# zhou-lab/biscuit

Measured on AMD Instinct MI355X. Metric: paired-end reads aligned/sec, higher is better.
Workload: dtype int32

## Files before the change

biscuit_amd/csrc/hip/k_swl.hip:

```cpp
#include <hip/hip_runtime.h>
#include "dev_common.hpp"
#include "wave.hpp"
#include "kernels.h"

#define SWL_ROW_ROR(n) (0x120 + (n))
__device__ __forceinline__ int swl_shl1(int v) { return __builtin_amdgcn_update_dpp(0, v, DPP_ROW_SHR(1), 0xf, 0xf, false); }
__device__ __forceinline__ int swl_row_max(int v)
{
	int t;
	t = __builtin_amdgcn_update_dpp(v, v, SWL_ROW_ROR(1), 0xf, 0xf, false); v = v > t ? v : t;
	t = __builtin_amdgcn_update_dpp(v, v, SWL_ROW_ROR(2), 0xf, 0xf, false); v = v > t ? v : t;
	t = __builtin_amdgcn_update_dpp(v, v, SWL_ROW_ROR(4), 0xf, 0xf, false); v = v > t ? v : t;
	t = __builtin_amdgcn_update_dpp(v, v, SWL_ROW_ROR(8), 0xf, 0xf, false); v = v > t ? v : t;
	return v;
}
__device__ __forceinline__ int swl_row_min(int v)
{
	int t;
	t = __builtin_amdgcn_update_dpp(v, v, SWL_ROW_ROR(1), 0xf, 0xf, false); v = v < t ? v : t;
	t = __builtin_amdgcn_update_dpp(v, v, SWL_ROW_ROR(2), 0xf, 0xf, false); v = v < t ? v : t;
	t = __builtin_amdgcn_update_dpp(v, v, SWL_ROW_ROR(4), 0xf, 0xf, false); v = v < t ? v : t;
	t = __builtin_amdgcn_update_dpp(v, v, SWL_ROW_ROR(8), 0xf, 0xf, false); v = v < t ? v : t;
	return v;
}
__device__ __forceinline__ unsigned int swl_row_or(unsigned int v)
{
	v |= (unsigned int)__builtin_amdgcn_update_dpp((int)v, (int)v, SWL_ROW_ROR(1), 0xf, 0xf, false);
	v |= (unsigned int)__builtin_amdgcn_update_dpp((int)v, (int)v, SWL_ROW_ROR(2), 0xf, 0xf, false);
	v |= (unsigned int)__builtin_amdgcn_update_dpp((int)v, (int)v, SWL_ROW_ROR(4), 0xf, 0xf, false);
	v |= (unsigned int)__builtin_amdgcn_update_dpp((int)v, (int)v, SWL_ROW_ROR(8), 0xf, 0xf, false);
	return v;
}
__device__ __forceinline__ int swl_clamp(int v, int hi) { return v < 0 ? 0 : v > hi ? hi : v; }

template <int SL, bool UNI>
__device__ __forceinline__ int swl_row(int (&H)[SL], int (&E)[SL], const uint32_t (&prof)[SL], int tsh, int cap, int slen,
                                       int oe_del, int e_del, int oe_ins, int e_ins, int col0_e)
{
	int f = 0, mxv = 0, hlast = 0, gl = NEG_BIG, ce = col0_e;
#pragma unroll
	for (int j = 0; j < SL; ++j) hlast = j == slen - 1 ? H[j] : hlast;
	int h = swl_shl1(hlast);
#pragma unroll
	for (int j = 0; j < SL; ++j) {
		if (j < slen) {
			const int s = (int)(int8_t)(prof[j] >> tsh);
			h = swl_clamp(h + s, cap);
			int e = E[j];
			h = h > e ? h : e;
			h = h > f ? h : f;
			mxv = mxv > h ? mxv : h;
			const int hold = H[j];
			H[j] = h;
			e -= e_del;
			int t = h - oe_del;
			e = e > t ? e : t;
			E[j] = e > 0 ? e : 0;
			f -= e_ins;
			t = h - oe_ins;
			f = f > t ? f : t;
			f = f > 0 ? f : 0;
			t += ce; gl = gl > t ? gl : t;
			ce += e_ins;
			h = hold;
		}
	}
	int t;
	t = __builtin_amdgcn_update_dpp(NEG_BIG, gl, DPP_ROW_SHR(1), 0xf, 0xf, false); gl = gl > t ? gl : t;
	t = __builtin_amdgcn_update_dpp(NEG_BIG, gl, DPP_ROW_SHR(2), 0xf, 0xf, false); gl = gl > t ? gl : t;
	t = __builtin_amdgcn_update_dpp(NEG_BIG, gl, DPP_ROW_SHR(4), 0xf, 0xf, false); gl = gl > t ? gl : t;
	t = __builtin_amdgcn_update_dpp(NEG_BIG, gl, DPP_ROW_SHR(8), 0xf, 0xf, false); gl = gl > t ? gl : t;
	int v = __builtin_amdgcn_update_dpp(NEG_BIG, gl, DPP_ROW_SHR(1), 0xf, 0xf, false) - (col0_e - e_ins);
	if (__ballot(v > 0) != 0) {
#pragma unroll
		for (int j = 0; j < SL; ++j) {
			if (j < slen) { H[j] = H[j] > v ? H[j] : v; v -= e_ins; }
		}
	}
	return mxv;
}

template <int SL>
__global__ void __launch_bounds__(256)
k_swl(DevIndex ix, DevScoring sc, const uint8_t *reads, const bsx_sw_job_t *jobs, const int *order, long long n,
      bsx_sw_res_t *res, unsigned long long *bscratch, int bcap)
{
	const int lane = wave_lane(), g = lane >> 4, k = lane & 15;
	const long long wave_id = (long long)blockIdx.x * (blockDim.x >> 6) + (threadIdx.x >> 6), n_waves = (long long)gridDim.x * (blockDim.x >> 6);
	unsigned long long *b = bscratch + ((size_t)wave_id * 4 + g) * (size_t)bcap;
	const int oe_del = sc.o_del + sc.e_del, oe_ins = sc.o_ins + sc.e_ins, e_del = sc.e_del, e_ins = sc.e_ins;
	for (long long q4 = wave_id; q4 * 4 < n; q4 += n_waves) {
		const long long jj = q4 * 4 + g;
		const bool valid = jj < n;
		const int job = valid ? order[jj] : 0;
		bsx_sw_job_t J = jobs[valid ? job : order[0]];
		const int8_t *mat = J.use_ct ? sc.ctmat : sc.gamat;
		int shift = 127, mx = 0;
		for (int a = 0; a < 25; ++a) { const int m = mat[a]; shift = m < shift ? m : shift; mx = m > mx ? m : mx; }
		shift = (int)(uint8_t)(256 - (int)(uint8_t)shift);
		const int cap = 255 - shift;
		bsx_sw_res_t o;
		o.score = 0; o.te = -1; o.qe = -1; o.score2 = -1; o.te2 = -1; o.tb = -1; o.qb = -1;
		int r_score = 0, r_te = -1, r_qe = -1;
		bool run = valid;
		for (int pass = 0; pass < 2; ++pass) {
			const int qlen = pass ? r_qe + 1 : J.qlen, tlen = J.tlen, te_rev = pass ? r_te : -1;
			const int xtra = pass ? (BSX_KSW_XSTOP | r_score) : J.xtra;
			const int minsc = (xtra & BSX_KSW_XSUBO) ? (xtra & 0xffff) : 0x10000;
			const int endsc = (xtra & BSX_KSW_XSTOP) ? (xtra & 0xffff) : 0x10000;
			const int slen = (qlen + 15) >> 4;
			const int slen_s = __builtin_amdgcn_readfirstlane(wave_max_i32(run ? slen : 0));
			const bool uni = __ballot(run && slen != slen_s) == 0;
			int H[SL], E[SL], Hm[SL];
			uint32_t prof[SL];
#pragma unroll
			for (int j = 0; j < SL; ++j) {
				H[j] = E[j] = Hm[j] = 0;
				const int c = j + k * slen;
				int q = 5;
				if (run && j < slen && c < qlen) {
					q = pass ? reads[(long long)J.qoff + (long long)(r_qe - c) * J.qdir] : reads[(long long)J.qoff + (long long)c * J.qdir];
					if (J.qcomp) q = q < 4 ? 3 - q : 4;
				}
				prof[j] = q > 4 ? 0u : ((uint32_t)(uint8_t)mat[q] | (uint32_t)(uint8_t)mat[5 + q] << 8 | (uint32_t)(uint8_t)mat[10 + q] << 16 | (uint32_t)(uint8_t)mat[15 + q] << 24);
			}
			int gmax = 0, te = -1, n_b = 0;
			unsigned long long b_last = 0;
			unsigned int tw = 0;
			bool live = run && tlen > 0;
			int rows = live ? tlen : 0;
			rows = wave_max_i32(rows);
			for (int i = 0; i < rows; ++i) {
				if (!__builtin_amdgcn_readfirstlane(__ballot(live) != 0)) break;
				if (live && i >= tlen) live = false;
				if (live) {
					if ((i & 15) == 0) {
						const int ii = i + k;
						const long long src = (ii <= te_rev) ? (long long)(te_rev - ii) : (long long)ii;
						const unsigned int tb = ii < tlen ? (unsigned int)dev_ref_base(ix.pac, ix.l_pac, J.tpos + src * J.tdir) : 0u;
						tw = swl_row_or(tb << (k << 1));
					}
					const int tsh = (int)((tw >> ((i & 15) << 1)) & 3u) << 3;
					int mxv;
					if (uni) mxv = swl_row<SL, true>(H, E, prof, tsh, cap, slen_s, oe_del, e_del, oe_ins, e_ins, k * slen_s * e_ins);
					else mxv = swl_row<SL, false>(H, E, prof, tsh, cap, slen, oe_del, e_del, oe_ins, e_ins, k * slen * e_ins);
					const int imax = swl_row_max(mxv);
					if (imax >= minsc) {
						if (n_b == 0 || (int)(uint32_t)b_last + 1 != i) { b_last = (unsigned long long)imax << 32 | (uint32_t)i; ++n_b; }
						else if ((int)(b_last >> 32) < imax) b_last = (unsigned long long)imax << 32 | (uint32_t)i;
						if (k == 0) b[n_b - 1] = b_last;
					}
					if (imax > gmax) {
						gmax = imax; te = i;
#pragma unroll
						for (int j = 0; j < SL; ++j) Hm[j] = H[j];
						if (gmax + shift >= 255 || gmax >= endsc) live = false;
					}
				}
			}
			const int score = gmax + shift < 255 ? gmax : 255;
			int qe = -1, score2 = -1, te2 = -1;
			if (run && score != 255) {
				int lm = -1, lj = 0x7fffffff;
#pragma unroll
				for (int j = 0; j < SL; ++j) if (j < slen) { const int c = j + k * slen; if (Hm[j] > lm || (Hm[j] == lm && c < lj)) { lm = Hm[j]; lj = c; } }
				const int m = swl_row_max(lm);
				qe = swl_row_min(lm == m ? lj : 0x7fffffff);
				if (n_b > 0) {
					WAVE_SYNC();
					const int rad = (score + mx - 1) / mx, low = te - rad, high = te + rad;
					int bs = -1, bi = 0x7fffffff;
					for (int x = k; x < n_b; x += 16) {
						const unsigned long long v = b[x];
						const int e = (int)(uint32_t)v, s2 = (int)(v >> 32);
						if ((e < low || e > high) && s2 > bs) { bs = s2; bi = x; }
					}
					const int ms = swl_row_max(bs);
					if (ms >= 0) {
						const int mi = swl_row_min(bs == ms ? bi : 0x7fffffff);
						score2 = ms; te2 = (int)(uint32_t)b[mi];
					}
					WAVE_SYNC();
				}
			}
			if (pass == 0) {
				o.score = score; o.te = te; o.qe = qe; o.score2 = score2; o.te2 = te2;
				r_score = score; r_te = te; r_qe = qe;
				run = run && (J.xtra & BSX_KSW_XSTART) && !((J.xtra & BSX_KSW_XSUBO) && score < (J.xtra & 0xffff)) && qe >= 0;
				if (__ballot(run) == 0) break;
			} else if (run && r_score == score) { o.tb = r_te - te; o.qb = r_qe - qe; }
		}
		if (valid && k == 0) res[job] = o;
	}
}

void launch_swl(hipStream_t st, const DevIndex &ix, const DevScoring &sc, const uint8_t *reads, const bsx_sw_job_t *jobs, const int *order,
                long long n, bsx_sw_res_t *res, unsigned long long *bscratch, int bcap, int blocks, int slen_max)
{
	if (slen_max <= 10) hipLaunchKernelGGL((k_swl<10>), dim3(blocks), dim3(256), 0, st, ix, sc, reads, jobs, order, n, res, bscratch, bcap);
	else hipLaunchKernelGGL((k_swl<16>), dim3(blocks), dim3(256), 0, st, ix, sc, reads, jobs, order, n, res, bscratch, bcap);
}
```

biscuit_amd/csrc/hip/kernels.h:

```cpp
#pragma once
#include <hip/hip_runtime.h>
#include "dev_common.hpp"
#include "seed_core.hpp"
#include "seed_tab.hpp"
#include "ctr_layout.hpp"

void launch_seed(hipStream_t st, int grid, const DevIndex &ix, const uint8_t *reads, const bsx_seed_task_t *tasks, int n_tasks, const SeedParams &P,
                 DevIntv *scratch, int list_cap, int mem_cap, DevIntv *out, unsigned long long out_cap, unsigned long long *out_cursor,
                 long long *task_off, int *task_n, unsigned int *task_cursor, unsigned long long *counters,
                 int quota, unsigned int *slab_busy, int n_slabs, int trip_budget, int prof = 0, uint32_t *qpack = nullptr, unsigned long long direct_off = ~0ull);
void launch_seedt(hipStream_t st, int grid, const DevIndex &ix, const uint8_t *reads, const bsx_seed_task_t *tasks, int n_tasks, const SeedParams &P,
                  DevIntv *scratch, int list_cap, int mem_cap, DevIntv *out, unsigned long long out_cap, unsigned long long *out_cursor,
                  long long *task_off, int *task_n, unsigned int *task_cursor, unsigned long long *counters,
                  int quota, unsigned int *slab_busy, int n_slabs, int trip_budget, int prof = 0, uint32_t *qpack = nullptr, unsigned long long direct_off = ~0ull);
size_t seedt_pack_bytes(long long n_tasks);
void launch_gather_lists(hipStream_t st, const DevIntv *src, const long long *off, const int *cnt, const long long *which, const long long *dst_off, long long n_list, DevIntv *dst);
int seedtab_build(hipStream_t st, const DevIndex &ix, int parent, int K, void *table);
void launch_bwt_planes(hipStream_t st, uint32_t *bwt, unsigned long long n_words);
void launch_sa(hipStream_t st, int grid, const DevIndex &ix, const bsx_sa_job_t *jobs, long long n, uint64_t *pos, unsigned long long *counters);
void launch_extend(hipStream_t st, const DevIndex &ix, const DevScoring &sc, const uint8_t *reads, const bsx_ext_job_t *jobs, const int *order,
                   long long n, bsx_ext_res_t *res, int qcap, int nc, int n_cu);
size_t extend_hbm_row_bytes(int qcap);
void launch_extend_hbm(hipStream_t st, const DevIndex &ix, const DevScoring &sc, const uint8_t *reads, const bsx_ext_job_t *jobs, const int *order,
                       long long n, bsx_ext_res_t *res, int qcap, int blocks, void *rows);
size_t global_hbm_row_bytes(int qcap);
void launch_global_hbm(hipStream_t st, const DevIndex &ix, const DevScoring &sc, const uint8_t *reads, const bsx_glb_job_t *jobs, const int *order,
                       long long n, bsx_glb_res_t *res, uint32_t *pool, uint8_t *zscratch, size_t zstride, int qcap, int blocks,
                       bsx_glb_tag_t *tags, char *md_pool, unsigned long long md_cap, unsigned long long *md_cursor, void *rows, bsx_glb_ctx_t *ctx = nullptr);
void launch_sw(hipStream_t st, const DevIndex &ix, const DevScoring &sc, const uint8_t *reads, const bsx_sw_job_t *jobs, const int *order,
               long long n, bsx_sw_res_t *res, unsigned long long *bscratch, int bcap, int blocks, int nc);
void launch_swl(hipStream_t st, const DevIndex &ix, const DevScoring &sc, const uint8_t *reads, const bsx_sw_job_t *jobs, const int *order,
                long long n, bsx_sw_res_t *res, unsigned long long *bscratch, int bcap, int blocks, int slen_max);
void launch_global(hipStream_t st, const DevIndex &ix, const DevScoring &sc, const uint8_t *reads, const bsx_glb_job_t *jobs, const int *order,
                   long long n, bsx_glb_res_t *res, uint32_t *pool, uint8_t *zscratch, size_t zstride, int qcap, int nc, int blocks, int wpb,
                   bsx_glb_tag_t *tags = nullptr, char *md_pool = nullptr, unsigned long long md_cap = 0, unsigned long long *md_cursor = nullptr, int tcap = 0,
                   bsx_glb_ctx_t *ctx = nullptr);
void launch_qc(hipStream_t st, const DevIndex &ix, const uint8_t *reads, long long reads_len, const bsx_qc_job_t *jobs, long long n, const uint32_t *pool,
               unsigned long long *table, int n_cu);
#define COV_LDS_BINS_MAX 512
size_t cov_n_tiles(long long l_pac);
size_t cov_diff_entries(long long l_pac);
size_t cov_mask_words(long long l_pac);
void launch_cov_add(hipStream_t st, int n_cu, void *diff, long long l_pac, const bsx_qc_job_t *jobs, long long n, const uint32_t *pool, long long pool_len);
void launch_cov_paint(hipStream_t st, int n_cu, uint32_t *mask, long long l_pac, const long long *beg_end, long long n);
void launch_cov_sums(hipStream_t st, int n_cu, const void *diff, long long n_tiles, void *tsum);
void launch_cov_max(hipStream_t st, int n_cu, const DevIndex &ix, const void *diff, const void *carry, long long n_tiles, int *gmax);
void launch_cov_count(hipStream_t st, int n_cu, const DevIndex &ix, const void *diff, const void *carry, long long n_tiles, const uint32_t *m_top,
                      const uint32_t *m_bot, int lds_bins, int flush_tiles, unsigned long long *bins, long long nb);
#define METH_FLUSH_TILES_MAX 1024
size_t meth_n_tiles(long long l_pac);
size_t meth_state_entries(long long l_pac);
void launch_meth_add(hipStream_t st, const DevIndex &ix, const uint8_t *reads, long long reads_len, const bsx_meth_job_t *jobs, long long n,
                     const uint32_t *pool, long long pool_len, void *state, int n_cu);
void launch_meth_tables(hipStream_t st, int n_cu, const DevIndex &ix, const void *state, long long n_tiles, int flush_tiles, unsigned long long *out);
struct MdSlot { unsigned long long claim, ord, k0, k1; };
enum { MD_CTR_TAKEN = 0, MD_CTR_OPEN = 1, MD_CTR_LOST = 2 };
enum { MD_RES_FIRST = 0, MD_RES_DUP = 1, MD_RES_OPEN = 2, MD_RES_SKIP = 3, MD_RES_FULL = 4 };
void launch_md_init(hipStream_t st, MdSlot *T, unsigned long long n_slots);
void launch_md_round(hipStream_t st, MdSlot *T, unsigned long long n_slots, const bsx_markdup_key_t *keys, long long n, unsigned long long first,
                     unsigned salt, int bits, uint8_t *res, unsigned long long *slot, unsigned long long *ctr);
void launch_md_rehash(hipStream_t st, const MdSlot *old, unsigned long long n_old, MdSlot *T, unsigned long long n_slots, unsigned long long *ctr);
#define SORT_SCAN_BLOCK 2048
size_t sort_n_tiles(long long n);
size_t sort_n_scan_blocks(long long n);
void launch_sort_bits(hipStream_t st, const unsigned long long *keys, long long n, unsigned long long *bits);
// ... 75 lines not shown
```

biscuit_amd/csrc/hip/shim.hip:

```cpp
#include <hip/hip_runtime.h>
#include <stdio.h>
#include <stdlib.h>
#include <string.h>
#include <time.h>
#include <algorithm>
#include <vector>
#include <mutex>
#include <atomic>
#include "devbuf.hpp"
#include "kernels.h"
#include "index_build.h"
#include "tune.h"
#include "ext_pk_bound.h"

#define HIPCHK(x) do { hipError_t e_ = (x); if (e_ != hipSuccess) { fprintf(stderr, "[bsx-hip] %s failed: %s (%s:%d)\n", #x, hipGetErrorString(e_), __FILE__, __LINE__); return BSX_E_NODEVICE; } } while (0)

#define BSX_LANES 6
enum KTime { KT_SEED = 0, KT_K3 = 1, KT_EXTEND = 2, KT_SW = 3, KT_GLOBAL = 4, KT_TIER1 = 5, KT_TIERS_LATER = 6, KT_SEED_OTHER = 7, KT_N = 8 };
struct Lane {
	hipStream_t st = nullptr;
	hipEvent_t ev_seed_done = nullptr, ev_regions_done = nullptr;
	hipStream_t st_hi = nullptr;
	hipEvent_t ev_timed_begin = nullptr, ev_timed_end = nullptr;
	hipEvent_t ev_seed2_begin = nullptr, ev_seed2_end = nullptr;
// ... 1583 lines not shown
		else if (!launch_swl16_batch(L.st_hi, d->n_cu, d->ix, L.sc, (const uint8_t*)L.reads.p, (const bsx_sw_job_t*)L.jobs.p, (bsx_sw_res_t*)L.res.p, (unsigned int)n, L.scratch.p))
			return BSX_E_ARG;
		HIPCHK(hipGetLastError());
		D2H(L.st_hi, res, L.res.p, (size_t)n * sizeof(bsx_sw_res_t));
		return BSX_OK;
	}
	std::vector<int> order[4];
	int max_tlen = 1, slen_max = 1;
	const bool use_swl = true;
	std::vector<int> key;
	for (int64_t i = 0; i < n; ++i) {
		const bsx_sw_job_t &j = jobs[i];
		if (j.qlen <= 0 || j.tlen < 0) { fprintf(stderr, "[bsx-hip] sw job %lld: invalid\n", (long long)i); return BSX_E_ARG; }
		const int p = (j.xtra & BSX_KSW_XBYTE) ? 16 : 8, Q = (j.qlen + p - 1) / p * p;
		if (Q > 3072) { fprintf(stderr, "[bsx-hip] sw job %lld: query %d beyond kernel limit (3072)\n", (long long)i, j.qlen); return BSX_E_ARG; }
		max_tlen = std::max(max_tlen, j.tlen);
		if (use_swl && p == 16 && Q <= 256) { order[3].push_back((int)i); slen_max = std::max(slen_max, Q / 16); }
		else order[Q <= 256 ? 0 : Q <= 1024 ? 1 : 2].push_back((int)i);
	}
	if (order[3].size() > 4) {
		const int NK = 17 * 2048;
		std::vector<int> cnt((size_t)NK + 1, 0), sorted(order[3].size());
		auto keyof = [&](int i) { const bsx_sw_job_t &j = jobs[i]; return ((j.qlen + 15) >> 4) * 2048 + (2047 - std::min(j.tlen, 2047)); };
		for (int i : order[3]) ++cnt[(size_t)keyof(i) + 1];
		for (int x = 0; x < NK; ++x) cnt[(size_t)x + 1] += cnt[(size_t)x];
		for (int i : order[3]) sorted[(size_t)cnt[(size_t)keyof(i)]++] = i;
		order[3].swap(sorted);
	}
	int rc;
	const int blocks_cap = d->n_cu * 8;
	if ((rc = L.jobs.reserve((size_t)n * sizeof(bsx_sw_job_t))) != BSX_OK) return rc;
	if ((rc = L.res.reserve((size_t)n * sizeof(bsx_sw_res_t))) != BSX_OK) return rc;
	if ((rc = L.aux.reserve((size_t)n * 4 + 64)) != BSX_OK) return rc;
	if ((rc = L.scratch.reserve((size_t)blocks_cap * 4 * 4 * (size_t)max_tlen * 8)) != BSX_OK) return rc;
	const bool tr_sw = bsx_phases() != 0;
	const double ts0 = tr_sw ? bsx_now_s() : 0;
	H2D(L.st_hi, L.jobs.p, jobs, (size_t)n * sizeof(bsx_sw_job_t));
	size_t off = 0;
	for (int c = 0; c < 4; ++c) if (!order[c].empty()) {
		H2D(L.st_hi, (int*)L.aux.p + off, order[c].data(), order[c].size() * 4);
		off += order[c].size();
	}
	HIPCHK(hipEventRecord(L.ev_timed_begin, L.st_hi));
	off = 0;
	for (int c = 0; c < 4; ++c) if (!order[c].empty()) {
		const long long m = (long long)order[c].size();
		if (c == 3) {
			const int blocks = (int)std::min<long long>((m + 15) / 16, blocks_cap);
			launch_swl(L.st_hi, d->ix, L.sc, (const uint8_t*)L.reads.p, (const bsx_sw_job_t*)L.jobs.p, (const int*)L.aux.p + off, m,
			           (bsx_sw_res_t*)L.res.p, (unsigned long long*)L.scratch.p, max_tlen, blocks, slen_max);
		} else {
			const int blocks = (int)std::min<long long>((m + 3) / 4, blocks_cap);
			launch_sw(L.st_hi, d->ix, L.sc, (const uint8_t*)L.reads.p, (const bsx_sw_job_t*)L.jobs.p, (const int*)L.aux.p + off, m,
			          (bsx_sw_res_t*)L.res.p, (unsigned long long*)L.scratch.p, max_tlen, blocks, c == 0 ? 4 : c == 1 ? 16 : 48);
		}
		off += order[c].size();
	}
	HIPCHK(hipEventRecord(L.ev_timed_end, L.st_hi));
	const double ts1 = tr_sw ? bsx_now_s() : 0;
	if ((rc = finish_timed(L, KT_SW)) != BSX_OK) return rc;
	const double ts2 = tr_sw ? bsx_now_s() : 0;
	D2H(L.st_hi, res, L.res.p, (size_t)n * sizeof(bsx_sw_res_t));
	if (tr_sw) { float ms = 0; (void)hipEventElapsedTime(&ms, L.ev_timed_begin, L.ev_timed_end);
		fprintf(stderr, "[M::sw_batch] %lld jobs: upload %.3f s, waited %.3f s for the kernels (%.3f s on the device), download %.3f s\n", (long long)n, ts1 - ts0, ts2 - ts1, ms * 1e-3, bsx_now_s() - ts2); }
	return BSX_OK;
}

static int lane_regions_dedup(bsx_device_t *d, int lane, const bsx_opt_t *opt, int64_t n_reads, int per_read, int32_t *out_n, uint8_t *out_idx,
                              int64_t *long_off = nullptr, uint16_t **long_idx = nullptr, int64_t *long_cap = nullptr)
{
	if (!d || !d->has_index) return BSX_E_NODEVICE;
	if (!opt || !out_n || !out_idx || per_read < 1) return BSX_E_ARG;
	Lane &L = d->lane[lane];
	if (n_reads == 0) return BSX_OK;
	if (n_reads * per_read != L.rb_tasks) { fprintf(stderr, "[bsx-hip] regions_dedup: %lld reads x %d strand searches, but the last regions batch had %lld\n", (long long)n_reads, per_read, (long long)L.rb_tasks); return BSX_E_ARG; }
	HIPCHK(hipSetDevice(d->ordinal));
	int rc;
	const int64_t n = L.rb_tasks;
	const size_t cap = (size_t)dedup_cap();
	const bool with_long = long_off && long_idx && long_cap && per_read <= 4 && bsx_tune_long("long_dedup", 1) != 0;
	const size_t pool_cap = with_long ? (size_t)L.rs.used_main + 64 : 0;
	const size_t o_idx = (size_t)n_reads * 4, o_list = (o_idx + (size_t)n_reads * cap + 15) & ~(size_t)15, o_off = o_list + (size_t)n_reads * 8, o_cnt = o_off + (size_t)n_reads * 8, o_pool = o_cnt + 16;
	if ((rc = L.dd.reserve(with_long ? o_pool + pool_cap * 2 + 64 : o_idx + (size_t)n_reads * cap + 64)) != BSX_OK) return rc;
// ... 36 lines not shown
	if (p1 <= p0) { *n_jobs = 0; return BSX_OK; }
	if (!bsx_tune_long("msw_plan", 0)) return BSX_OK;
	if (!L.ddl.valid || L.ddl.n_reads != n_reads || L.ddl.per_read != per_read || n_reads * per_read != L.rb_tasks) return BSX_OK;
	if (max_len <= 0 || max_len > 256 || (long long)max_len * opt->a >= 250 || opt->max_matesw > 64 || opt->max_matesw < 1 || (opt->flag & BSX_F_SELF_OVLP)) return BSX_OK;
	std::lock_guard<std::mutex> hi_lock(L.hi_mu);
	HIPCHK(hipSetDevice(d->ordinal));
	int rc;
	const int np = p1 - p0, MM = opt->max_matesw;
	const size_t job_cap = (size_t)np * 2 * (size_t)MM;
	const size_t tb = (size_t)np * msw_pair_bytes(), o_hist = (tb + 255) & ~(size_t)255, o_cnt = o_hist + (size_t)msw_hist_bins() * 4, o_ord = o_cnt + 256;
	if ((rc = L.msw_jobs.reserve(job_cap * sizeof(bsx_sw_job_t) + 64)) != BSX_OK) return rc;
	if ((rc = L.msw_res.reserve(job_cap * sizeof(bsx_sw_res_t) + 64)) != BSX_OK) return rc;
	if ((rc = L.msw_meta.reserve(o_ord + job_cap * 4 + 64)) != BSX_OK) return rc;
	if (L.msw_token != token) {
		if ((rc = L.msw_roff.reserve(((size_t)n_reads + 1) * 4)) != BSX_OK) return rc;
		H2D(L.st_hi, L.msw_roff.p, roff, ((size_t)n_reads + 1) * 4);
		L.msw_token = token;
	}
	char *M = (char*)L.msw_meta.p;
	unsigned int *d_hist = (unsigned int*)(M + o_hist), *d_cnt = (unsigned int*)(M + o_cnt);
	int *d_ord = (int*)(M + o_ord);
	HIPCHK(hipMemsetAsync(d_hist, 0, (size_t)msw_hist_bins() * 4 + 256, L.st_hi));
	const int64_t n = L.rb_tasks;
	const long long *r_off = (const long long*)L.regmeta.p; const int *r_n = (const int*)((const char*)L.regmeta.p + (size_t)n * 8);
	const char *DD = (const char*)L.dd.p;
	launch_msw_plan(L.st_hi, d->n_cu, d->ix, (const bsx_region_t*)L.regs.p, r_off, r_n, (const int*)DD, (const unsigned char*)DD + L.ddl.o_idx,
	                L.ddl.with_long ? (const long long*)(DD + L.ddl.o_off) : nullptr, L.ddl.with_long ? (const unsigned short*)(DD + L.ddl.o_pool) : nullptr, dedup_cap(), per_read,
	                (const unsigned int*)L.msw_roff.p, pes->low, pes->high, opt->pen_unpaired, MM, opt->min_seed_len, opt->a, p0, np,
	                (bsx_sw_job_t*)L.msw_jobs.p, (unsigned int)std::min<size_t>(job_cap, 0xfffffff0u), d_cnt, d_hist, M, d_ord);
	unsigned int nj = 0;
	D2H(L.st_hi, &nj, d_cnt, 4);
	if ((size_t)nj > job_cap) nj = (unsigned int)job_cap;
	if (nj) {
		const int blocks_cap = d->n_cu * 8;
		long long bound = (long long)pes->high - (long long)pes->low + max_len + 8;
		if (bound < 1) bound = 1;
		if (bound > (1 << 20)) { *n_jobs = -1; return BSX_OK; }
		if ((rc = L.scratch.reserve((size_t)blocks_cap * 4 * 4 * (size_t)bound * 8)) != BSX_OK) return rc;
		const int blocks = (int)std::min<long long>(((long long)nj + 15) / 16, blocks_cap);
		HIPCHK(hipEventRecord(L.ev_timed_begin, L.st_hi));
		launch_swl(L.st_hi, d->ix, L.sc, (const uint8_t*)L.reads.p, (const bsx_sw_job_t*)L.msw_jobs.p, (const int*)d_ord, (long long)nj,
		           (bsx_sw_res_t*)L.msw_res.p, (unsigned long long*)L.scratch.p, (int)bound, blocks, (max_len + 15) / 16);
		HIPCHK(hipEventRecord(L.ev_timed_end, L.st_hi));
		if ((rc = finish_timed(L, KT_SW)) != BSX_OK) return rc;
		if (*res_cap < (int64_t)nj) { *res_cap = (int64_t)nj + (nj >> 2) + 1024; *res = (bsx_sw_res_t*)realloc(*res, sizeof(bsx_sw_res_t) * (size_t)*res_cap); }
		D2H(L.st_hi, *res, L.msw_res.p, (size_t)nj * sizeof(bsx_sw_res_t));
	}
	D2H(L.st_hi, table, M, tb);
	HIPCHK(hipGetLastError());
	*n_jobs = (int64_t)nj;
	if (bsx_phases()) fprintf(stderr, "[M::msw_plan] pairs %d..%d: %u alignments planned and run on the device\n", p0, p1, nj);
	return BSX_OK;
}

static int lane_global_batch(bsx_device_t *d, int lane, int64_t n, const bsx_glb_job_t *jobs, bsx_glb_res_t *res,
                             uint32_t *cigar_pool, size_t cigar_pool_len, bsx_glb_tag_t *tags = nullptr, char **md = nullptr, int64_t *md_cap = nullptr,
                             bsx_glb_ctx_t *ctx = nullptr)
{
	if (!d || !d->has_index) return BSX_E_NODEVICE;
	Lane &L = d->lane[lane];
	if (n == 0) return BSX_OK;
	std::lock_guard<std::mutex> hi_lock(L.hi_mu);
	HIPCHK(hipSetDevice(d->ordinal));
	static const int QCAP[4] = {256, 1024, 16384, 0x7fffffff}, BAND[4] = {256, 1024, 2048, 2048}, NCS[4] = {4, 16, 32, 32}, WPB[4] = {4, 4, 1, 1};
	std::vector<int> order[4];
	size_t zmax[4] = {64, 64, 64, 64};
	int hbm_qmax = 0;
	static const int TCAP[4] = {512, 2048, 0, 0};
	size_t md_bound = 64;
	const DevScoring &sc = L.sc;
	for (int64_t i = 0; i < n; ++i) {
		const bsx_glb_job_t &j = jobs[i];
		if (tags && j.want_cigar) md_bound += 2 * (size_t)j.tlen + 16;
		if (j.qlen <= 0 || j.tlen <= 0 || j.n_try < 1) { fprintf(stderr, "[bsx-hip] global job %lld: invalid\n", (long long)i); return BSX_E_ARG; }
		if (j.want_cigar && (size_t)j.cigar_off + j.cigar_cap > cigar_pool_len) return BSX_E_ARG;
// ... 717 lines not shown
```

biscuit_amd/csrc/host/tune.c:

```c
#include <pthread.h>
#include "bsx_core.h"
#include "tune.h"

typedef struct { const char *name, *doc; char *val; } knob_t;
static knob_t g_knobs[] = {
	{"phases", "[0] 1: per-phase lines on stderr and the kernels' cycle counters; 2: the stage counters read after every region launch (also $BSX_PHASES)", 0},
	{"tiers", "[0] 1: HIP events between the region launches of a chunk, printed (no cycle counters): bench.py's stand-alone chunk", 0},
	{"seed_form", "[table] classic: seeding without the table of k-mer intervals (k_seed.hip: the reference's own sequence of bwt_extend calls, what counts its FM-block touches)", 0},
	{"seed_tab_k", "[from the text's size: 18 at 3.1 Gbp] levels of the table of k-mer intervals; 0: none", 0},
	{"seed_mem_cap", "[max(64, longest read)] entries of a strand search's first-pass interval list (tests: short lists, so that ordinary reads are seeded again)", 0},
	{"seed_direct", "[1] 0: interval lists copied behind each other instead of written where they stay", 0},
	{"seed_batch_form", "[batch] chunk: bsx_seed_batch launches as the chunk-wide seeding pass of bsx_regions_batch does (its list length, lists written where they stay, budget, quota, grid and slabs; what is left seeded again with lists eight times as long) -- tests: the production launch, list for list", 0},
	{"seed_quota", "[0 = persistent lanes; 1 for seed_form=classic] strand searches a lane of the seeding kernel takes", 0},
	{"tier3_early", "[1] the last HBM tier's launch for what is known to need it when the occurrences are counted: on a stream of its own beside the other tiers; 0: behind them", 0},
	{"tier3_order", "[1] the last HBM tier takes its strand searches longest first (by occurrences to visit); 0: in the order the tier before handed them on", 0},
	{"tier3_wgs", "[2] workgroups of four waves per CU in the last HBM tier's launch (1..3)", 0},
	{"seed_budget2", "[8] the second seeding pass's budget in first-pass budgets; what exceeds it is seeded a third time on the side stream, without one", 0},
	{"seed_trip_budget", "[4096] FM extensions (per 256 bases of read) after which the first seeding pass hands a strand search to the second; 0: never", 0},
	{"redo_merge_min", "[4096] from how many overflowed strand searches the second seeding pass runs inside the chunk's launch sequence (1: always; negative or huge: never)", 0},
	{"async_redo", "[0] 1: bsx_process_seqs collects the strand searches seeded again on the side stream only in the back half", 0},
	{"device_sa_intv", "[2] the device's suffix-array sample: every n-th rank (a power of two up to the files' 32)", 0},
	{"pos_cap", "[384 per strand search] seed occurrences the chunk-wide position table holds (tests: strand searches that find no room)", 0},
	{"ssw_cap", "[24 per strand search] jobs the seed filter's chunk-wide list holds (tests: seeds that find no room)", 0},
	{"regions_quota", "[16] strand searches per wave of the first region tier", 0},
	{"mid_quota", "[8] strand searches per wave of the larger LDS tiers", 0},
	{"c2r_quota", "[16] strand searches per wave of the chains -> regions launch", 0},
	{"regions_occ", "[5] waves per SIMD the first region tier's register allocation targets (3..5)", 0},
	{"regions_mid", "[1] 0: no second LDS tier", 0},
	{"tier1c", "[1] 0: no third LDS tier / second chains -> regions launch for ordinary reads (the tier sequence of rounds 2-4)", 0},
	{"x4", "[1] 0: every extension inline in the chains -> regions loop (no k_x4prep / k_extl / k_ext4 ahead of it)", 0},
	{"xl", "[1] 0: the narrow extension jobs through k_ext4 as well (no lane-per-job kernel)", 0},
	{"ext_win", "[1] chunks with long reads: an extension's rows in five register slots that follow the band (ext_dp_win); 0: in LDS (the form of rounds 3-5)", 0},
	{"ext4", "[off] tests: bsx_extend_batch through the quarter-wave kernel (1) / then the lane-per-job kernel (2) of the regions path / through the wavefront-per-job form with a register window (3) / with the rows of the region kernels' inline extensions, packed 16-bit when the batch allows (4)", 0},
	{"sw_form", "[off] tests: bsx_sw_batch through the seed filter's alignments, score only, jobs of up to 199 x 199 in the order given -- ssw16: the packed 16-bit kernel (k_swl16), sixteen consecutive jobs to a wavefront, qlen = 0 an empty job; scoring options it cannot hold fail the call / ssw32: a wavefront per job through the 32-bit alignment of a seed without room in the job list", 0},
	{"ext_pk", "[1] extension rows of 64 columns and more in packed 16-bit, two columns per lane (ext_pk.hpp), where the scoring options keep every intermediate inside 16 bits; 0: always the 32-bit rows", 0},
	{"chain_stages", "[3] how consecutive chunks' front halves are chained on the device: 0 none, 1 seeding, 2 seeding and regions, 3 the same but the HBM tiers hold nobody back, 4 strictly one after the other", 0},
	{"small_copies_unmasked", "[1] the front half's copies of less than 256 KB go through the lane's unmasked stream (the CUs the front-half streams leave alone); 0: through the stream they are ordered on", 0},
	{"reserve_cu_every", "[0] n >= 2: the front-half streams leave one compute unit in n (of every shader engine of every XCD) to the back half's short batches; < 2: none", 0},
	{"host_chain", "[0] 1: every strand search chained on the host over the batch kernels (A/B against the region kernels)", 0},
	{"host_dedup", "[0] 1: mem_sort_deduplicate of every read on the host (A/B against k_dedup)", 0},
	{"stream_whole_chunk", "[0] N: a chunk's own thread runs its back half too, at most N at a time", 0},
	{"no_chunk_scan", "[0] 1 (several ranks): no boundary scan of plain input files, every rank parses everything", 0},
	{"no_chunk_skip", "[0] 1 (several ranks): the other ranks' chunks are parsed into records and dropped instead of walked", 0},
	{"index_batch", "[256 M] suffixes per batch of the device index builder's first round", 0},
	{"back_slices", "[4] slices the pairs of a chunk are cut into for the stages after the insert-size statistics (mate rescue .. SAM text); 1: the stages over the whole chunk", 0},
	{"back_threads", "[2] threads that take those slices alternately (one waits for its slice's K5 / K6 batch while the other runs host stages); up to 4", 0},
	{"shard_pairs", "[0] several ranks (RANK / WORLD_SIZE): 1 = every rank aligns its slice of EVERY chunk (inputs with fewer chunks than GPUs) instead of every world-th chunk", 0},
	{"gather_via_rank0", "[0] several ranks with $BSX_OUT: 1 = the records go through rank 0 even where every rank could write its own chunks into the file", 0},
	{"gather_transport", "[rccl] several ranks: socket = Unix-domain sockets through rank 0 instead of RCCL", 0},
	{"tier2_export", "[0] the first HBM tier of the region kernels in steps -- chains exported, seeds extended ahead (k_extl / k_ext4; 1: every chain's best seed, 2: every seed of every main list), the seed loop by a chains -> regions launch with its regions in HBM -- instead of its monolithic form (same SAM; measured no faster, DESIGN.md section 4)", 0},
	{"msw_plan", "[0] 1: mate rescue's plan pass (which candidates need an alignment, over which window) by k_msw_plan over the lists on the device, its K5 batch run from device memory, instead of by the host's first replay pass (same SAM; measured slower, DESIGN.md section 4)", 0},
	{"long_dedup", "[1] 0: reads with more than 32 regions are de-duplicated on the host (A/B against k_dedup_long)", 0},
	{"markdup_slots", "[32 per key of the first batch, at least 65536] slots of the first table of template keys (--markdup), a power of two; it doubles before a batch would load it beyond one half", 0},
	{"cov_lds_bins", "[512] depths below this are counted in a workgroup's LDS histograms by the coverage tables' last pass (--qc-cov), deeper ones in HBM directly; a power of two up to 512", 0},
	{"meth_flush_tiles", "[1024] tests: tiles after which a wave of the base-averaged conversion table's pass (--qc-meth) adds its sums to the 64-bit cells (32-bit registers: at most 1024)", 0},
	{"cov_flush_tiles", "[524287] tests: tiles after which a workgroup of that pass adds its LDS histograms to the bins (32-bit cells: at most 2^32 / 4096 - 1)", 0},
	{"sort_buf_bytes", "[1 GB / runs, at most 8 MB] bytes of the buffer every sorted run of --sort is read back through in the final merge (tests: 1, a record is then many fills)", 0},
	{"markdup_hash_bits", "[64] tests: low bits kept of a template key's claim word (different keys then meet in one slot and take the next salt)", 0},
};
#define N_KNOBS ((int)(sizeof(g_knobs) / sizeof(g_knobs[0])))
static pthread_mutex_t g_mu = PTHREAD_MUTEX_INITIALIZER;
static int g_env_done = 0, g_phases_env = -1;

static int find(const char *name)
{
	int i;
	for (i = 0; i < N_KNOBS; ++i) if (strcmp(g_knobs[i].name, name) == 0) return i;
// ... 70 lines not shown
```

Measured before the change: 730,100.

## Make byte-mode SW kernel persistent with atomic job cursor and per-group state machine

```diff
diff --git a/biscuit_amd/csrc/hip/k_swl.hip b/biscuit_amd/csrc/hip/k_swl.hip
--- a/biscuit_amd/csrc/hip/k_swl.hip
+++ b/biscuit_amd/csrc/hip/k_swl.hip
@@ -1,9 +1,13 @@
 #include <hip/hip_runtime.h>
+#include <algorithm>
 #include "dev_common.hpp"
 #include "wave.hpp"
 #include "kernels.h"
+#include "tune.h"
 
 #define SWL_ROW_ROR(n) (0x120 + (n))
+#define SWL_TAKE 16u
+#define SWL_HEAD 256
 __device__ __forceinline__ int swl_shl1(int v) { return __builtin_amdgcn_update_dpp(0, v, DPP_ROW_SHR(1), 0xf, 0xf, false); }
 __device__ __forceinline__ int swl_row_max(int v)
 {
@@ -33,11 +37,11 @@
 }
 __device__ __forceinline__ int swl_clamp(int v, int hi) { return v < 0 ? 0 : v > hi ? hi : v; }
 
-template <int SL, bool UNI>
+template <int SL, bool UNI, bool EQG>
 __device__ __forceinline__ int swl_row(int (&H)[SL], int (&E)[SL], const uint32_t (&prof)[SL], int tsh, int cap, int slen,
-                                       int oe_del, int e_del, int oe_ins, int e_ins, int col0_e)
-{
-	int f = 0, mxv = 0, hlast = 0, gl = NEG_BIG, ce = col0_e;
+                                       int oe_del, int e_del, int oe_ins, int e_ins, int end_e)
+{
+	int f = 0, mxv = 0, hlast = 0;
 #pragma unroll
 	for (int j = 0; j < SL; ++j) hlast = j == slen - 1 ? H[j] : hlast;
 	int h = swl_shl1(hlast);
@@ -53,24 +57,22 @@
 			const int hold = H[j];
 			H[j] = h;
 			e -= e_del;
-			int t = h - oe_del;
+			const int t = h - oe_del;
 			e = e > t ? e : t;
 			E[j] = e > 0 ? e : 0;
 			f -= e_ins;
-			t = h - oe_ins;
-			f = f > t ? f : t;
+			const int u = EQG ? t : h - oe_ins;
+			f = f > u ? f : u;
 			f = f > 0 ? f : 0;
-			t += ce; gl = gl > t ? gl : t;
-			ce += e_ins;
 			h = hold;
 		}
 	}
-	int t;
+	int gl = f + end_e, t;
 	t = __builtin_amdgcn_update_dpp(NEG_BIG, gl, DPP_ROW_SHR(1), 0xf, 0xf, false); gl = gl > t ? gl : t;
 	t = __builtin_amdgcn_update_dpp(NEG_BIG, gl, DPP_ROW_SHR(2), 0xf, 0xf, false); gl = gl > t ? gl : t;
 	t = __builtin_amdgcn_update_dpp(NEG_BIG, gl, DPP_ROW_SHR(4), 0xf, 0xf, false); gl = gl > t ? gl : t;
 	t = __builtin_amdgcn_update_dpp(NEG_BIG, gl, DPP_ROW_SHR(8), 0xf, 0xf, false); gl = gl > t ? gl : t;
-	int v = __builtin_amdgcn_update_dpp(NEG_BIG, gl, DPP_ROW_SHR(1), 0xf, 0xf, false) - (col0_e - e_ins);
+	int v = __builtin_amdgcn_update_dpp(NEG_BIG, gl, DPP_ROW_SHR(1), 0xf, 0xf, false) - (end_e - slen * e_ins);
 	if (__ballot(v > 0) != 0) {
 #pragma unroll
 		for (int j = 0; j < SL; ++j) {
@@ -80,123 +82,206 @@
 	return mxv;
 }
 
-template <int SL>
+enum { SWL_IDLE = 0, SWL_SETUP, SWL_ROW, SWL_AFTER, SWL_DONE };
+
+template <int SL, bool EQG>
 __global__ void __launch_bounds__(256)
-k_swl(DevIndex ix, DevScoring sc, const uint8_t *reads, const bsx_sw_job_t *jobs, const int *order, long long n,
-      bsx_sw_res_t *res, unsigned long long *bscratch, int bcap)
-{
-	const int lane = wave_lane(), g = lane >> 4, k = lane & 15;
-	const long long wave_id = (long long)blockIdx.x * (blockDim.x >> 6) + (threadIdx.x >> 6), n_waves = (long long)gridDim.x * (blockDim.x >> 6);
+k_swl(DevIndex ix, DevScoring sc, const uint8_t *reads, const bsx_sw_job_t *jobs, const int *order, unsigned int n,
+      bsx_sw_res_t *res, unsigned long long *bscratch, int bcap, unsigned int *cursor, int n_waves)
+{
+	__shared__ uint32_t s_sqp[2][8];
+	__shared__ int s_shift[2], s_mx[2];
+	if (threadIdx.x < 16) {
+		const int p = threadIdx.x >> 3, q = threadIdx.x & 7;
+		const int8_t *mat = p ? sc.ctmat : sc.gamat;
+		s_sqp[p][q] = q > 4 ? 0u : ((uint32_t)(uint8_t)mat[q] | (uint32_t)(uint8_t)mat[5 + q] << 8 | (uint32_t)(uint8_t)mat[10 + q] << 16 | (uint32_t)(uint8_t)mat[15 + q] << 24);
+		if (q == 0) {
+			int shift = 127, mx = 0;
+			for (int a = 0; a < 25; ++a) { const int m = mat[a]; shift = m < shift ? m : shift; mx = m > mx ? m : mx; }
+			s_shift[p] = (int)(uint8_t)(256 - (int)(uint8_t)shift);
+			s_mx[p] = mx;
+		}
+	}
+	__syncthreads();
+	const int lane = wave_lane(), g = lane >> 4, k = lane & 15, gsh = lane & 48;
+	const int wave_id = (int)(blockIdx.x * (blockDim.x >> 6) + (threadIdx.x >> 6));
+	if (wave_id >= n_waves) return;
 	unsigned long long *b = bscratch + ((size_t)wave_id * 4 + g) * (size_t)bcap;
 	const int oe_del = sc.o_del + sc.e_del, oe_ins = sc.o_ins + sc.e_ins, e_del = sc.e_del, e_ins = sc.e_ins;
-	for (long long q4 = wave_id; q4 * 4 < n; q4 += n_waves) {
-		const long long jj = q4 * 4 + g;
-		const bool valid = jj < n;
-		const int job = valid ? order[jj] : 0;
-		bsx_sw_job_t J = jobs[valid ? job : order[0]];
-		const int8_t *mat = J.use_ct ? sc.ctmat : sc.gamat;
-		int shift = 127, mx = 0;
-		for (int a = 0; a < 25; ++a) { const int m = mat[a]; shift = m < shift ? m : shift; mx = m > mx ? m : mx; }
-		shift = (int)(uint8_t)(256 - (int)(uint8_t)shift);
-		const int cap = 255 - shift;
-		bsx_sw_res_t o;
-		o.score = 0; o.te = -1; o.qe = -1; o.score2 = -1; o.te2 = -1; o.tb = -1; o.qb = -1;
-		int r_score = 0, r_te = -1, r_qe = -1;
-		bool run = valid;
-		for (int pass = 0; pass < 2; ++pass) {
-			const int qlen = pass ? r_qe + 1 : J.qlen, tlen = J.tlen, te_rev = pass ? r_te : -1;
-			const int xtra = pass ? (BSX_KSW_XSTOP | r_score) : J.xtra;
-			const int minsc = (xtra & BSX_KSW_XSUBO) ? (xtra & 0xffff) : 0x10000;
-			const int endsc = (xtra & BSX_KSW_XSTOP) ? (xtra & 0xffff) : 0x10000;
-			const int slen = (qlen + 15) >> 4;
-			const int slen_s = __builtin_amdgcn_readfirstlane(wave_max_i32(run ? slen : 0));
-			const bool uni = __ballot(run && slen != slen_s) == 0;
-			int H[SL], E[SL], Hm[SL];
-			uint32_t prof[SL];
-#pragma unroll
-			for (int j = 0; j < SL; ++j) {
-				H[j] = E[j] = Hm[j] = 0;
-				const int c = j + k * slen;
-				int q = 5;
-				if (run && j < slen && c < qlen) {
-					q = pass ? reads[(long long)J.qoff + (long long)(r_qe - c) * J.qdir] : reads[(long long)J.qoff + (long long)c * J.qdir];
-					if (J.qcomp) q = q < 4 ? 3 - q : 4;
+	const long long l_pac = ix.l_pac;
+	int st = SWL_IDLE, wait = 0, pass = 0;
+	unsigned int wnext = 0, wend = 0; bool wdone = false;
+	int job = 0, mi = 0;
+	bsx_sw_job_t J; J.tpos = 0; J.qoff = 0; J.qlen = J.tlen = J.xtra = 0; J.qdir = J.tdir = 1; J.qcomp = J.use_ct = 0;
+	bsx_sw_res_t o; o.score = 0; o.te = o.qe = o.score2 = o.te2 = o.tb = o.qb = -1;
+	int qlen = 0, te_rev = -1, minsc = 0, endsc = 0, slen = 1, end_e = 0, shift = 0, cap = 0;
+	int i = 0, gmax = 0, te = -1, n_b = 0;
+	unsigned long long b_last = 0;
+	unsigned int tw = 0, tbn = 0;
+	int H[SL], E[SL], Hm[SL];
+	uint32_t prof[SL];
+#pragma unroll
+	for (int j = 0; j < SL; ++j) { H[j] = E[j] = Hm[j] = 0; prof[j] = 0; }
+	auto bases = [&](int i0) -> unsigned int {
+		const int ii = i0 + k;
+		const long long src = (ii <= te_rev) ? (long long)(te_rev - ii) : (long long)ii;
+		const unsigned int tb = ii < J.tlen ? (unsigned int)dev_ref_base(ix.pac, l_pac, J.tpos + src * J.tdir) : 0u;
+		return tb << (k << 1);
+	};
+	for (;;) {
+		{
+			const bool cold = st != SWL_ROW && st != SWL_DONE;
+			const unsigned long long cm = __ballot(cold), rm = __ballot(st == SWL_ROW);
+			if (cold) ++wait;
+			if (cm && (rm == 0 || __popcll(cm) >= 32 || __ballot(wait >= 3))) {
+				if (st == SWL_AFTER) {
+					const int score = gmax + shift < 255 ? gmax : 255;
+					int qe = -1, score2 = -1, te2 = -1;
+					if (score != 255) {
+						int lm = -1, lj = 0x7fffffff;
+#pragma unroll
+						for (int j = 0; j < SL; ++j) if (j < slen) { const int c = j + k * slen; if (Hm[j] > lm || (Hm[j] == lm && c < lj)) { lm = Hm[j]; lj = c; } }
+						const int m = swl_row_max(lm);
+						qe = swl_row_min(lm == m ? lj : 0x7fffffff);
+						if (n_b > 0) {
+							WAVE_SYNC();
+							const int mx = s_mx[mi];
+							const int rad = (score + mx - 1) / mx, low = te - rad, high = te + rad;
+							int bs = -1, bi = 0x7fffffff;
+							for (int x = k; x < n_b; x += 16) {
+								const unsigned long long v = b[x];
+								const int e = (int)(uint32_t)v, s2 = (int)(v >> 32);
+								if ((e < low || e > high) && s2 > bs) { bs = s2; bi = x; }
+							}
+							const int ms = swl_row_max(bs);
+							if (ms >= 0) {
+								const int at = swl_row_min(bs == ms ? bi : 0x7fffffff);
+								score2 = ms; te2 = (int)(uint32_t)b[at];
+							}
+							WAVE_SYNC();
+						}
+					}
+					bool again = false;
+					if (pass == 0) {
+						o.score = score; o.te = te; o.qe = qe; o.score2 = score2; o.te2 = te2;
+						again = (J.xtra & BSX_KSW_XSTART) && !((J.xtra & BSX_KSW_XSUBO) && score < (J.xtra & 0xffff)) && qe >= 0;
+					} else if (o.score == score) { o.tb = o.te - te; o.qb = o.qe - qe; }
+					if (again) { pass = 1; st = SWL_SETUP; }
+					else { if (k == 0) res[job] = o; st = SWL_IDLE; }
 				}
-				prof[j] = q > 4 ? 0u : ((uint32_t)(uint8_t)mat[q] | (uint32_t)(uint8_t)mat[5 + q] << 8 | (uint32_t)(uint8_t)mat[10 + q] << 16 | (uint32_t)(uint8_t)mat[15 + q] << 24);
+				for (int rep = 0; rep < 2; ++rep) {
+					const unsigned long long need = __ballot(st == SWL_IDLE);
+					if (need == 0) break;
+					const unsigned long long heads = need & 0x0001000100010001ull;
+					if (wnext == wend && !wdone) {
+						unsigned int base = 0;
+						if (lane == 0) base = atomicAdd(cursor, SWL_TAKE);
+						base = (unsigned int)__builtin_amdgcn_readfirstlane((int)base);
+						wnext = base < n ? base : n; wend = base + SWL_TAKE < n ? base + SWL_TAKE : n;
+						if (wnext == wend) wdone = true;
+					}
+					const unsigned int e_new = wnext + (unsigned int)__popcll(heads & ((1ull << gsh) - 1));
+					const bool served = e_new < wend;
+					wnext = wnext + (unsigned int)__popcll(heads) < wend ? wnext + (unsigned int)__popcll(heads) : wend;
+					if (st == SWL_IDLE) {
+						if (!served) { if (wdone) st = SWL_DONE; }
+						else {
+							job = order[e_new];
+							J = jobs[job];
+							mi = J.use_ct ? 1 : 0;
+							shift = s_shift[mi]; cap = 255 - shift;
+							o.score = 0; o.te = o.qe = o.score2 = o.te2 = o.tb = o.qb = -1;
+							pass = 0; st = SWL_SETUP;
+						}
+					}
+				}
+				if (st == SWL_SETUP) {
+					qlen = pass ? o.qe + 1 : J.qlen; te_rev = pass ? o.te : -1;
+					const int xtra = pass ? (BSX_KSW_XSTOP | o.score) : J.xtra;
+					minsc = (xtra & BSX_KSW_XSUBO) ? (xtra & 0xffff) : 0x10000;
+					endsc = (xtra & BSX_KSW_XSTOP) ? (xtra & 0xffff) : 0x10000;
+					slen = (qlen + 15) >> 4;
+					end_e = (k * slen + slen - 1) * e_ins;
+#pragma unroll
+					for (int j = 0; j < SL; ++j) {
+						H[j] = E[j] = Hm[j] = 0;
+						const int c = j + k * slen;
+						int q = 5;
+						if (j < slen && c < qlen) {
+							q = pass ? reads[(long long)J.qoff + (long long)(o.qe - c) * J.qdir] : reads[(long long)J.qoff + (long long)c * J.qdir];
+							if (J.qcomp) q = q < 4 ? 3 - q : 4;
+							q = q < 5 ? q : 5;
+						}
+						prof[j] = s_sqp[mi][q];
+					}
+					gmax = 0; te = -1; n_b = 0; b_last = 0; i = 0;
+					if (J.tlen > 0) { tbn = bases(0); st = SWL_ROW; }
+					else st = SWL_AFTER;
+				}
+				if (st == SWL_ROW || st == SWL_DONE) wait = 0;
 			}
-			int gmax = 0, te = -1, n_b = 0;
-			unsigned long long b_last = 0;
-			unsigned int tw = 0;
-			bool live = run && tlen > 0;
-			int rows = live ? tlen : 0;
-			rows = wave_max_i32(rows);
-			for (int i = 0; i < rows; ++i) {
-				if (!__builtin_amdgcn_readfirstlane(__ballot(live) != 0)) break;
-				if (live && i >= tlen) live = false;
-				if (live) {
-					if ((i & 15) == 0) {
-						const int ii = i + k;
-						const long long src = (ii <= te_rev) ? (long long)(te_rev - ii) : (long long)ii;
-						const unsigned int tb = ii < tlen ? (unsigned int)dev_ref_base(ix.pac, ix.l_pac, J.tpos + src * J.tdir) : 0u;
-						tw = swl_row_or(tb << (k << 1));
-					}
-					const int tsh = (int)((tw >> ((i & 15) << 1)) & 3u) << 3;
-					int mxv;
-					if (uni) mxv = swl_row<SL, true>(H, E, prof, tsh, cap, slen_s, oe_del, e_del, oe_ins, e_ins, k * slen_s * e_ins);
-					else mxv = swl_row<SL, false>(H, E, prof, tsh, cap, slen, oe_del, e_del, oe_ins, e_ins, k * slen * e_ins);
-					const int imax = swl_row_max(mxv);
-					if (imax >= minsc) {
-						if (n_b == 0 || (int)(uint32_t)b_last + 1 != i) { b_last = (unsigned long long)imax << 32 | (uint32_t)i; ++n_b; }
-						else if ((int)(b_last >> 32) < imax) b_last = (unsigned long long)imax << 32 | (uint32_t)i;
-						if (k == 0) b[n_b - 1] = b_last;
-					}
-					if (imax > gmax) {
-						gmax = imax; te = i;
-#pragma unroll
-						for (int j = 0; j < SL; ++j) Hm[j] = H[j];
-						if (gmax + shift >= 255 || gmax >= endsc) live = false;
-					}
-				}
+			if (__ballot(st == SWL_ROW) == 0) { if (__ballot(st != SWL_DONE) == 0) break; continue; }
+		}
+		const bool run = st == SWL_ROW;
+		int slen_s, uni;
+		{
+			const int sv = run ? slen : 0;
+			const int s0 = __builtin_amdgcn_readlane(sv, 0), s1 = __builtin_amdgcn_readlane(sv, 16), s2 = __builtin_amdgcn_readlane(sv, 32), s3 = __builtin_amdgcn_readlane(sv, 48);
+			const int m01 = s0 > s1 ? s0 : s1, m23 = s2 > s3 ? s2 : s3;
+			slen_s = m01 > m23 ? m01 : m23;
+			uni = (s0 == 0 || s0 == slen_s) && (s1 == 0 || s1 == slen_s) && (s2 == 0 || s2 == slen_s) && (s3 == 0 || s3 == slen_s);
+		}
+		if (run) {
+			if ((i & 15) == 0) { tw = swl_row_or(tbn); tbn = bases(i + 16); }
+			const int tsh = (int)((tw >> ((i & 15) << 1)) & 3u) << 3;
+			int mxv;
+			if (uni) mxv = swl_row<SL, true, EQG>(H, E, prof, tsh, cap, slen_s, oe_del, e_del, oe_ins, e_ins, end_e);
+			else mxv = swl_row<SL, false, EQG>(H, E, prof, tsh, cap, slen, oe_del, e_del, oe_ins, e_ins, end_e);
+			const int imax = swl_row_max(mxv);
+			bool stop = false;
+			if (imax >= minsc) {
+				if (n_b == 0 || (int)(uint32_t)b_last + 1 != i) { b_last = (unsigned long long)imax << 32 | (uint32_t)i; ++n_b; }
+				else if ((int)(b_last >> 32) < imax) b_last = (unsigned long long)imax << 32 | (uint32_t)i;
+				if (k == 0) b[n_b - 1] = b_last;
 			}
-			const int score = gmax + shift < 255 ? gmax : 255;
-			int qe = -1, score2 = -1, te2 = -1;
-			if (run && score != 255) {
-				int lm = -1, lj = 0x7fffffff;
-#pragma unroll
-				for (int j = 0; j < SL; ++j) if (j < slen) { const int c = j + k * slen; if (Hm[j] > lm || (Hm[j] == lm && c < lj)) { lm = Hm[j]; lj = c; } }
-				const int m = swl_row_max(lm);
-				qe = swl_row_min(lm == m ? lj : 0x7fffffff);
-				if (n_b > 0) {
-					WAVE_SYNC();
-					const int rad = (score + mx - 1) / mx, low = te - rad, high = te + rad;
-					int bs = -1, bi = 0x7fffffff;
-					for (int x = k; x < n_b; x += 16) {
-						const unsigned long long v = b[x];
-						const int e = (int)(uint32_t)v, s2 = (int)(v >> 32);
-						if ((e < low || e > high) && s2 > bs) { bs = s2; bi = x; }
-					}
-					const int ms = swl_row_max(bs);
-					if (ms >= 0) {
-						const int mi = swl_row_min(bs == ms ? bi : 0x7fffffff);
-						score2 = ms; te2 = (int)(uint32_t)b[mi];
-					}
-					WAVE_SYNC();
-				}
+			if (imax > gmax) {
+				gmax = imax; te = i;
+#pragma unroll
+				for (int j = 0; j < SL; ++j) Hm[j] = H[j];
+				stop = gmax + shift >= 255 || gmax >= endsc;
 			}
-			if (pass == 0) {
-				o.score = score; o.te = te; o.qe = qe; o.score2 = score2; o.te2 = te2;
-				r_score = score; r_te = te; r_qe = qe;
-				run = run && (J.xtra & BSX_KSW_XSTART) && !((J.xtra & BSX_KSW_XSUBO) && score < (J.xtra & 0xffff)) && qe >= 0;
-				if (__ballot(run) == 0) break;
-			} else if (run && r_score == score) { o.tb = r_te - te; o.qb = r_qe - qe; }
-		}
-		if (valid && k == 0) res[job] = o;
-	}
-}
+			++i;
+			if (stop || i >= J.tlen) st = SWL_AFTER;
+		}
+	}
+}
+
+int swl_waves(int n_cu, long long n, int slen_max)
+{
+	static const int per_cu[2] = { [] { int nb = 0; return hipOccupancyMaxActiveBlocksPerMultiprocessor(&nb, k_swl<10, true>, 256, 0) == hipSuccess && nb > 0 ? nb * 4 : 8; }(),
+	                               [] { int nb = 0; return hipOccupancyMaxActiveBlocksPerMultiprocessor(&nb, k_swl<16, true>, 256, 0) == hipSuccess && nb > 0 ? nb * 4 : 8; }() };
+	long long w = (long long)n_cu * per_cu[slen_max <= 10 ? 0 : 1];
+	w = std::min(w, (n + 3) / 4);
+	const long cap = bsx_tune_long("swl_waves", 0);
+	if (cap > 0) w = std::min<long long>(w, cap);
+	return (int)std::max<long long>(w, 1);
+}
+size_t swl_scratch_bytes(int waves, int bcap) { return SWL_HEAD + (size_t)waves * 4 * (size_t)bcap * 8; }
 
 void launch_swl(hipStream_t st, const DevIndex &ix, const DevScoring &sc, const uint8_t *reads, const bsx_sw_job_t *jobs, const int *order,
-                long long n, bsx_sw_res_t *res, unsigned long long *bscratch, int bcap, int blocks, int slen_max)
-{
-	if (slen_max <= 10) hipLaunchKernelGGL((k_swl<10>), dim3(blocks), dim3(256), 0, st, ix, sc, reads, jobs, order, n, res, bscratch, bcap);
-	else hipLaunchKernelGGL((k_swl<16>), dim3(blocks), dim3(256), 0, st, ix, sc, reads, jobs, order, n, res, bscratch, bcap);
-}
+                long long n, bsx_sw_res_t *res, void *scratch, int bcap, int waves, int slen_max)
+{
+	unsigned int *cursor = (unsigned int*)scratch;
+	unsigned long long *b = (unsigned long long*)((char*)scratch + SWL_HEAD);
+	const bool eqg = sc.o_del + sc.e_del == sc.o_ins + sc.e_ins;
+	const dim3 grid((unsigned int)((waves + 3) / 4)), block(256);
+	const unsigned int nj = (unsigned int)n;
+	(void)hipMemsetAsync(cursor, 0, 4, st);
+	if (slen_max <= 10) {
+		if (eqg) hipLaunchKernelGGL((k_swl<10, true>), grid, block, 0, st, ix, sc, reads, jobs, order, nj, res, b, bcap, cursor, waves);
+		else hipLaunchKernelGGL((k_swl<10, false>), grid, block, 0, st, ix, sc, reads, jobs, order, nj, res, b, bcap, cursor, waves);
+	} else {
+		if (eqg) hipLaunchKernelGGL((k_swl<16, true>), grid, block, 0, st, ix, sc, reads, jobs, order, nj, res, b, bcap, cursor, waves);
+		else hipLaunchKernelGGL((k_swl<16, false>), grid, block, 0, st, ix, sc, reads, jobs, order, nj, res, b, bcap, cursor, waves);
+	}
+}
diff --git a/biscuit_amd/csrc/hip/kernels.h b/biscuit_amd/csrc/hip/kernels.h
--- a/biscuit_amd/csrc/hip/kernels.h
+++ b/biscuit_amd/csrc/hip/kernels.h
@@ -30,7 +30,9 @@
 void launch_sw(hipStream_t st, const DevIndex &ix, const DevScoring &sc, const uint8_t *reads, const bsx_sw_job_t *jobs, const int *order,
                long long n, bsx_sw_res_t *res, unsigned long long *bscratch, int bcap, int blocks, int nc);
 void launch_swl(hipStream_t st, const DevIndex &ix, const DevScoring &sc, const uint8_t *reads, const bsx_sw_job_t *jobs, const int *order,
-                long long n, bsx_sw_res_t *res, unsigned long long *bscratch, int bcap, int blocks, int slen_max);
+                long long n, bsx_sw_res_t *res, void *scratch, int bcap, int waves, int slen_max);
+int swl_waves(int n_cu, long long n, int slen_max);
+size_t swl_scratch_bytes(int waves, int bcap);
 void launch_global(hipStream_t st, const DevIndex &ix, const DevScoring &sc, const uint8_t *reads, const bsx_glb_job_t *jobs, const int *order,
                    long long n, bsx_glb_res_t *res, uint32_t *pool, uint8_t *zscratch, size_t zstride, int qcap, int nc, int blocks, int wpb,
                    bsx_glb_tag_t *tags = nullptr, char *md_pool = nullptr, unsigned long long md_cap = 0, unsigned long long *md_cursor = nullptr, int tcap = 0,
diff --git a/biscuit_amd/csrc/hip/shim.hip b/biscuit_amd/csrc/hip/shim.hip
--- a/biscuit_amd/csrc/hip/shim.hip
+++ b/biscuit_amd/csrc/hip/shim.hip
@@ -1639,7 +1639,9 @@
 	if ((rc = L.jobs.reserve((size_t)n * sizeof(bsx_sw_job_t))) != BSX_OK) return rc;
 	if ((rc = L.res.reserve((size_t)n * sizeof(bsx_sw_res_t))) != BSX_OK) return rc;
 	if ((rc = L.aux.reserve((size_t)n * 4 + 64)) != BSX_OK) return rc;
-	if ((rc = L.scratch.reserve((size_t)blocks_cap * 4 * 4 * (size_t)max_tlen * 8)) != BSX_OK) return rc;
+	const int swl_w = order[3].empty() ? 0 : swl_waves(d->n_cu, (long long)order[3].size(), slen_max);
+	const bool any_sw = !order[0].empty() || !order[1].empty() || !order[2].empty();
+	if ((rc = L.scratch.reserve(std::max(any_sw ? (size_t)blocks_cap * 4 * (size_t)max_tlen * 8 : (size_t)0, swl_w ? swl_scratch_bytes(swl_w, max_tlen) : (size_t)0))) != BSX_OK) return rc;
 	const bool tr_sw = bsx_phases() != 0;
 	const double ts0 = tr_sw ? bsx_now_s() : 0;
 	H2D(L.st_hi, L.jobs.p, jobs, (size_t)n * sizeof(bsx_sw_job_t));
@@ -1653,9 +1655,8 @@
 	for (int c = 0; c < 4; ++c) if (!order[c].empty()) {
 		const long long m = (long long)order[c].size();
 		if (c == 3) {
-			const int blocks = (int)std::min<long long>((m + 15) / 16, blocks_cap);
 			launch_swl(L.st_hi, d->ix, L.sc, (const uint8_t*)L.reads.p, (const bsx_sw_job_t*)L.jobs.p, (const int*)L.aux.p + off, m,
-			           (bsx_sw_res_t*)L.res.p, (unsigned long long*)L.scratch.p, max_tlen, blocks, slen_max);
+			           (bsx_sw_res_t*)L.res.p, L.scratch.p, max_tlen, swl_w, slen_max);
 		} else {
 			const int blocks = (int)std::min<long long>((m + 3) / 4, blocks_cap);
 			launch_sw(L.st_hi, d->ix, L.sc, (const uint8_t*)L.reads.p, (const bsx_sw_job_t*)L.jobs.p, (const int*)L.aux.p + off, m,
@@ -1758,15 +1759,14 @@
 	D2H(L.st_hi, &nj, d_cnt, 4);
 	if ((size_t)nj > job_cap) nj = (unsigned int)job_cap;
 	if (nj) {
-		const int blocks_cap = d->n_cu * 8;
 		long long bound = (long long)pes->high - (long long)pes->low + max_len + 8;
 		if (bound < 1) bound = 1;
 		if (bound > (1 << 20)) { *n_jobs = -1; return BSX_OK; }
-		if ((rc = L.scratch.reserve((size_t)blocks_cap * 4 * 4 * (size_t)bound * 8)) != BSX_OK) return rc;
-		const int blocks = (int)std::min<long long>(((long long)nj + 15) / 16, blocks_cap);
+		const int swl_w = swl_waves(d->n_cu, (long long)nj, (max_len + 15) / 16);
+		if ((rc = L.scratch.reserve(swl_scratch_bytes(swl_w, (int)bound))) != BSX_OK) return rc;
 		HIPCHK(hipEventRecord(L.ev_timed_begin, L.st_hi));
 		launch_swl(L.st_hi, d->ix, L.sc, (const uint8_t*)L.reads.p, (const bsx_sw_job_t*)L.msw_jobs.p, (const int*)d_ord, (long long)nj,
-		           (bsx_sw_res_t*)L.msw_res.p, (unsigned long long*)L.scratch.p, (int)bound, blocks, (max_len + 15) / 16);
+		           (bsx_sw_res_t*)L.msw_res.p, L.scratch.p, (int)bound, swl_w, (max_len + 15) / 16);
 		HIPCHK(hipEventRecord(L.ev_timed_end, L.st_hi));
 		if ((rc = finish_timed(L, KT_SW)) != BSX_OK) return rc;
 		if (*res_cap < (int64_t)nj) { *res_cap = (int64_t)nj + (nj >> 2) + 1024; *res = (bsx_sw_res_t*)realloc(*res, sizeof(bsx_sw_res_t) * (size_t)*res_cap); }
diff --git a/biscuit_amd/csrc/host/tune.c b/biscuit_amd/csrc/host/tune.c
--- a/biscuit_amd/csrc/host/tune.c
+++ b/biscuit_amd/csrc/host/tune.c
@@ -33,6 +33,7 @@
 	{"ext_win", "[1] chunks with long reads: an extension's rows in five register slots that follow the band (ext_dp_win); 0: in LDS (the form of rounds 3-5)", 0},
 	{"ext4", "[off] tests: bsx_extend_batch through the quarter-wave kernel (1) / then the lane-per-job kernel (2) of the regions path / through the wavefront-per-job form with a register window (3) / with the rows of the region kernels' inline extensions, packed 16-bit when the batch allows (4)", 0},
 	{"sw_form", "[off] tests: bsx_sw_batch through the seed filter's alignments, score only, jobs of up to 199 x 199 in the order given -- ssw16: the packed 16-bit kernel (k_swl16), sixteen consecutive jobs to a wavefront, qlen = 0 an empty job; scoring options it cannot hold fail the call / ssw32: a wavefront per job through the 32-bit alignment of a seed without room in the job list", 0},
+	{"swl_waves", "[0 = as many as the device holds] tests: at most this many persistent waves in a launch of the byte-mode alignment kernel (k_swl) -- 1: one wave's four rows of lanes run through the whole job list, cursor block after cursor block", 0},
 	{"ext_pk", "[1] extension rows of 64 columns and more in packed 16-bit, two columns per lane (ext_pk.hpp), where the scoring options keep every intermediate inside 16 bits; 0: always the 32-bit rows", 0},
 	{"chain_stages", "[3] how consecutive chunks' front halves are chained on the device: 0 none, 1 seeding, 2 seeding and regions, 3 the same but the HBM tiers hold nobody back, 4 strictly one after the other", 0},
 	{"small_copies_unmasked", "[1] the front half's copies of less than 256 KB go through the lane's unmasked stream (the CUs the front-half streams leave alone); 0: through the stream they are ordered on", 0},
```

After: 714,700. 2.1% lower.
